# PaddlePaddle/PaddleNLP

Measured on NVIDIA H100. Metric: tokens/sec Llama-3.2-3B seq4096 bf16 pretrain step (global, all GPUs), higher is better.
Workload: dtype bf16

## Files before the change

paddlenlp_b200/csrc/gemm_wgmma.cu:

```cuda
#include "../../include/b200nlp.h"
#include <cstdlib>
#include <cstring>

#include "common.cuh"
#include "host_util.h"

namespace b200 {
namespace gemm {

constexpr int BN = 256;
constexpr int BK = 64;
constexpr int B_BYTES = BN * BK * 2;
constexpr int EPI_BOX = 64;
constexpr int EPI_BOX_BYTES = EPI_BOX * EPI_BOX * 2;
constexpr int EPI_BOX_F32 = 32;

template <int NWG>
struct Tile {
  static constexpr int BM = 64 * NWG;
  static constexpr int NUM_THREADS = 128 * (NWG + 1);
  static constexpr int A_BYTES = BM * BK * 2;
  static constexpr int STAGE_BYTES = A_BYTES + B_BYTES;
  static constexpr int STAGES = NWG == 2 ? 4 : 5;
  static constexpr int EPI_BYTES = NWG * 2 * EPI_BOX_BYTES;
  static constexpr int SMEM_BYTES = STAGES * STAGE_BYTES + EPI_BYTES + 256 + 1024;
};
static int tile_wgs(int64_t M) { return M <= 64 ? 1 : 2; }

struct Params {
  int M, N, K;
  int num_m_tiles, num_n_tiles;
  int epi_mode;
  int swiglu_inter;
  int gm;
  int split_k;
  int kb_per_split;
  const float* bias;
  bf16* c;
  int64_t ldc;
  const bf16* r;
  int64_t ldr;
  bf16* aux;
  int64_t ld_aux;
  float* ws;
};

__device__ __forceinline__ void fence_acc(float (&acc)[128]) {
#pragma unroll
  for (int i = 0; i < 128; ++i) asm volatile("" : "+f"(acc[i])::"memory");
}

__device__ __forceinline__ uint32_t epi_slot(uint32_t buf, int r, int jj, int lane) {
  return buf + r * 128 + ((jj ^ (r & 7)) << 4) + 4 * (lane & 3);
}
template <int KEEP>
__device__ __forceinline__ void epi_begin(int cw, bool leader) {
  if (leader) tma_store_wait_read<KEEP>();
  named_bar_sync(1 + cw, 128);
}
__device__ __forceinline__ void epi_end(int cw) {
  fence_proxy_async_smem();
  named_bar_sync(1 + cw, 128);
}
__device__ __forceinline__ uint32_t ld_pair(const bf16* base, int64_t ld, int row, int col, int M, int N) {
  if (row >= M || col >= N) return 0u;
  const bf16* src = base + static_cast<int64_t>(row) * ld + col;
  if (col + 1 < N) return *reinterpret_cast<const uint32_t*>(src);
  return static_cast<uint32_t>(__bfloat16_as_ushort(*src));
}
__device__ __forceinline__ void epi_prefetch(const CUtensorMap* tmC, const CUtensorMap* tmX, const Params& p, int n_blk, int row0) {
  for (int s = 0; s < BN / EPI_BOX; ++s) {
    const int col0 = n_blk * BN + EPI_BOX * s;
    if (col0 >= p.N) break;
    if (p.epi_mode == 1) {
      tma_prefetch_l2_2d(tmC, col0, row0);
    } else if (p.epi_mode == 2) {
      tma_prefetch_l2_2d(tmX, col0, row0);
    } else {
      tma_prefetch_l2_2d(tmX, col0, row0);
      tma_prefetch_l2_2d(tmX, p.swiglu_inter + col0, row0);
    }
  }
}

template <int NWG, bool A_MN, bool B_MN>
__global__ void __launch_bounds__(Tile<NWG>::NUM_THREADS, 1)
gemm_bf16_kernel(const __grid_constant__ CUtensorMap tmA, const __grid_constant__ CUtensorMap tmB,
                 const __grid_constant__ CUtensorMap tmC, const __grid_constant__ CUtensorMap tmX, const Params p) {
  using T = Tile<NWG>;
  constexpr int BM = T::BM, A_BYTES = T::A_BYTES, STAGE_BYTES = T::STAGE_BYTES, STAGES = T::STAGES;
  extern __shared__ uint8_t smem_raw[];
  uint8_t* smem = reinterpret_cast<uint8_t*>((reinterpret_cast<uintptr_t>(smem_raw) + 1023) & ~uintptr_t(1023));
  uint64_t* full_bar = reinterpret_cast<uint64_t*>(smem + STAGES * STAGE_BYTES + T::EPI_BYTES);
  uint64_t* empty_bar = full_bar + STAGES;

  const int num_items = p.num_m_tiles * p.num_n_tiles * p.split_k;
  const int num_kb_total = (p.K + BK - 1) / BK;
  if (threadIdx.x == 0) {
    tma_prefetch_desc(&tmA);
    tma_prefetch_desc(&tmB);
    for (int i = 0; i < STAGES; ++i) {
      mbar_init(&full_bar[i], 1);
      mbar_init(&empty_bar[i], NWG * 128);
    }
    fence_mbar_init();
  }
  __syncthreads();
  pdl_launch_dependents();
  pdl_wait();

  const int wg = threadIdx.x >> 7;
  if (wg == 0) {
    setmaxnreg_dec<40>();
    if (threadIdx.x == 0) {
      uint32_t it = 0;
      for (int t = blockIdx.x; t < num_items; t += gridDim.x) {
        int m_blk, n_blk;
        tile_coords(t / p.split_k, p.num_m_tiles, p.num_n_tiles, m_blk, n_blk, p.gm);
        const int kb0 = (t % p.split_k) * p.kb_per_split;
        const int kb1 = min(num_kb_total, kb0 + p.kb_per_split);
        for (int kb = kb0; kb < kb1; ++kb, ++it) {
          const int st = static_cast<int>(it % STAGES);
          mbar_wait_nocall(&empty_bar[st], ((it / STAGES) & 1u) ^ 1u);
          uint8_t* sA = smem + st * STAGE_BYTES;
          uint8_t* sB = sA + A_BYTES;
          mbar_arrive_expect_tx(&full_bar[st], STAGE_BYTES);
          if constexpr (A_MN) {
#pragma unroll
            for (int h = 0; h < NWG; ++h) tma_load_2d(&tmA, &full_bar[st], sA + h * (64 * BK * 2), m_blk * BM + 64 * h, kb * BK);
          } else {
            tma_load_2d(&tmA, &full_bar[st], sA, kb * BK, m_blk * BM);
          }
          if constexpr (B_MN) {
#pragma unroll
            for (int h = 0; h < 4; ++h) {
              const int c0 = p.epi_mode == 4 ? (h >> 1) * p.swiglu_inter + n_blk * 128 + (h & 1) * 64 : n_blk * BN + h * 64;
              tma_load_2d(&tmB, &full_bar[st], sB + h * (B_BYTES / 4), c0, kb * BK);
            }
          } else {
            tma_load_2d(&tmB, &full_bar[st], sB, kb * BK, n_blk * BN);
            tma_load_2d(&tmB, &full_bar[st], sB + B_BYTES / 2, kb * BK, n_blk * BN + 128);
          }
        }
      }
    }
    return;
  }

  setmaxnreg_inc<232>();
  const int cw = wg - 1;
  const int wi = (threadIdx.x >> 5) & 3, lane = threadIdx.x & 31;
  const uint32_t ring = smem_u32(smem);
  constexpr uint32_t A_KSTEP = A_MN ? 2048u : 32u, B_KSTEP = B_MN ? 2048u : 32u;
  const uint32_t a_off = static_cast<uint32_t>(cw) * (64 * BK * 2);
  const bool leader = (threadIdx.x & 127) == 0;
  const bool prefetch = leader && (p.epi_mode == 1 || p.epi_mode == 2 || p.epi_mode == 5);
  const uint32_t ebuf = smem_u32(smem + STAGES * STAGE_BYTES) + cw * 2 * EPI_BOX_BYTES;
  uint32_t nbox = 0;
  uint32_t it = 0;
  float acc[128];
  for (int t = blockIdx.x; t < num_items; t += gridDim.x) {
    int m_blk, n_blk;
    tile_coords(t / p.split_k, p.num_m_tiles, p.num_n_tiles, m_blk, n_blk, p.gm);
    const int kb0 = (t % p.split_k) * p.kb_per_split;
    const int nkb = min(num_kb_total, kb0 + p.kb_per_split) - kb0;
    const int prefetch_kb = nkb > 8 ? nkb - 8 : 0;
    fence_acc(acc);
#pragma unroll
    for (int i = 0; i < 128; ++i) acc[i] = 0.f;
    fence_acc(acc);
    for (int i = 0; i < nkb; ++i, ++it) {
      const int st = static_cast<int>(it % STAGES);
      mbar_wait_nocall(&full_bar[st], (it / STAGES) & 1u);
      const uint32_t sA = ring + st * STAGE_BYTES + a_off, sB = ring + st * STAGE_BYTES + A_BYTES;
      const uint64_t dA = wgmma_desc_sw128(sA, A_MN ? 64 * BK * 2 : 16, 1024);
      const uint64_t dB = wgmma_desc_sw128(sB, B_MN ? B_BYTES / 4 : 16, 1024);
      wgmma_fence();
#pragma unroll
      for (int kk = 0; kk < BK / 16; ++kk)
        wgmma_m64n256k16<A_MN ? 1 : 0, B_MN ? 1 : 0>(acc, dA + ((kk * A_KSTEP) >> 4), dB + ((kk * B_KSTEP) >> 4),
                                                     (i > 0 || kk > 0) ? 1u : 0u);
      wgmma_commit();
      if (prefetch && i == prefetch_kb) epi_prefetch(&tmC, &tmX, p, n_blk, m_blk * BM + cw * 64);
      wgmma_wait<1>();
      if (i > 0) mbar_arrive(&empty_bar[(it - 1) % STAGES]);
    }
    wgmma_wait<0>();
    fence_acc(acc);
    if (nkb > 0) mbar_arrive(&empty_bar[(it - 1) % STAGES]);

    const int row0 = m_blk * BM + cw * 64;
    const int r_lo = wi * 16 + (lane >> 2);
    const int cq = 2 * (lane & 3);
    if (p.epi_mode == 3) {
#pragma unroll
      for (int i = 0; i < 2; ++i) {
        const int row = row0 + r_lo + 8 * i;
        if (row >= p.M) continue;
#pragma unroll
        for (int j = 0; j < 32; ++j) {
          const int col = n_blk * BN + 8 * j + cq;
          if (col >= p.N) continue;
          float* w = p.ws + static_cast<int64_t>(row) * p.N + col;
          asm volatile("red.global.add.v2.f32 [%0], {%1, %2};" ::"l"(w), "f"(acc[4 * j + 2 * i]), "f"(acc[4 * j + 2 * i + 1])
                       : "memory");
        }
      }
      continue;
    }
    if (p.epi_mode == 4) {
#pragma unroll
      for (int h = 0; h < 2; ++h) {
        const int ch0 = n_blk * 128 + EPI_BOX * h;
        if (ch0 >= p.swiglu_inter) continue;
        if (p.aux != nullptr) {
          epi_begin<0>(cw, leader);
#pragma unroll
          for (int i = 0; i < 2; ++i)
#pragma unroll
            for (int jj = 0; jj < 8; ++jj) {
              const int j = 8 * h + jj;
              st_shared_u32(epi_slot(ebuf, r_lo + 8 * i, jj, lane), pack_bf16x2(acc[4 * j + 2 * i], acc[4 * j + 2 * i + 1]));
              st_shared_u32(epi_slot(ebuf + EPI_BOX_BYTES, r_lo + 8 * i, jj, lane),
                            pack_bf16x2(acc[4 * (j + 16) + 2 * i], acc[4 * (j + 16) + 2 * i + 1]));
            }
          epi_end(cw);
          if (leader) {
            tma_store_2d(&tmX, ebuf, ch0, row0);
            tma_store_2d(&tmX, ebuf + EPI_BOX_BYTES, p.swiglu_inter + ch0, row0);
            tma_store_commit();
          }
        }
        epi_begin<0>(cw, leader);
#pragma unroll
        for (int i = 0; i < 2; ++i)
#pragma unroll
          for (int jj = 0; jj < 8; ++jj) {
            const int j = 8 * h + jj;
            const uint32_t gp = pack_bf16x2(acc[4 * j + 2 * i], acc[4 * j + 2 * i + 1]);
            const uint32_t up = pack_bf16x2(acc[4 * (j + 16) + 2 * i], acc[4 * (j + 16) + 2 * i + 1]);
            st_shared_u32(epi_slot(ebuf, r_lo + 8 * i, jj, lane), swiglu_fwd_pair(gp, up));
          }
        epi_end(cw);
        if (leader) {
          tma_store_2d(&tmC, ebuf, ch0, row0);
          tma_store_commit();
        }
      }
      continue;
    }
    if (p.epi_mode == 5) {
#pragma unroll
      for (int s = 0; s < BN / EPI_BOX; ++s) {
        const int ch0 = n_blk * BN + EPI_BOX * s;
        if (ch0 >= p.N) continue;
        epi_begin<0>(cw, leader);
#pragma unroll
        for (int q = 0; q < 4; ++q) {
          const int i = q >> 1, jj0 = 4 * (q & 1);
          uint32_t g[4], u[4];
#pragma unroll
          for (int k = 0; k < 4; ++k) {
            const int row = row0 + r_lo + 8 * i, ch = ch0 + 8 * (jj0 + k) + cq;
            g[k] = ld_pair(p.aux, p.ld_aux, row, ch, p.M, p.N);
            u[k] = ld_pair(p.aux + p.swiglu_inter, p.ld_aux, row, ch, p.M, p.N);
          }
#pragma unroll
          for (int k = 0; k < 4; ++k) {
            const int jj = jj0 + k, j = 8 * s + jj;
            uint32_t dg2, du2;
            swiglu_bwd_pair(g[k], u[k], bf16_round(acc[4 * j + 2 * i]), bf16_round(acc[4 * j + 2 * i + 1]), dg2, du2);
            st_shared_u32(epi_slot(ebuf, r_lo + 8 * i, jj, lane), dg2);
            st_shared_u32(epi_slot(ebuf + EPI_BOX_BYTES, r_lo + 8 * i, jj, lane), du2);
          }
        }
        epi_end(cw);
        if (leader) {
          tma_store_2d(&tmC, ebuf, ch0, row0);
          tma_store_2d(&tmC, ebuf + EPI_BOX_BYTES, p.swiglu_inter + ch0, row0);
          tma_store_commit();
        }
      }
      continue;
    }
#pragma unroll
    for (int s = 0; s < BN / EPI_BOX; ++s) {
      const int col0 = n_blk * BN + EPI_BOX * s;
      if (col0 >= p.N) continue;
      if (p.epi_mode >= 6) {
        const uint32_t sw = (lane >> 2) << 4;
        const uint32_t row_off = r_lo * 128 + ((8 * (lane & 3)) ^ (sw & 16));
        epi_begin<0>(cw, leader);
#pragma unroll
        for (int h = 0; h < 2; ++h)
#pragma unroll
          for (int jj = 0; jj < 4; ++jj) {
            const int j = 8 * s + 4 * h + jj;
            const uint32_t slot = ebuf + h * EPI_BOX_BYTES + row_off + ((32 * jj) ^ (sw & 96));
            st_shared_f32x2(slot, acc[4 * j], acc[4 * j + 1]);
            st_shared_f32x2(slot + 8 * 128, acc[4 * j + 2], acc[4 * j + 3]);
          }
        epi_end(cw);
        if (leader) {
          if (p.epi_mode == 7) {
            tma_reduce_add_2d(&tmC, ebuf, col0, row0);
            tma_reduce_add_2d(&tmC, ebuf + EPI_BOX_BYTES, col0 + EPI_BOX_F32, row0);
          } else {
            tma_store_2d(&tmC, ebuf, col0, row0);
            tma_store_2d(&tmC, ebuf + EPI_BOX_BYTES, col0 + EPI_BOX_F32, row0);
          }
          tma_store_commit();
        }
        continue;
      }
      const uint32_t buf = ebuf + (nbox++ & 1u) * EPI_BOX_BYTES;
      epi_begin<1>(cw, leader);
#pragma unroll
      for (int i = 0; i < 2; ++i) {
        uint32_t o[8];
        if (p.epi_mode != 0) {
          const bf16* src = p.epi_mode == 1 ? p.c : p.r;
          const int64_t ld = p.epi_mode == 1 ? p.ldc : p.ldr;
#pragma unroll
          for (int jj = 0; jj < 8; ++jj) o[jj] = ld_pair(src, ld, row0 + r_lo + 8 * i, col0 + 8 * jj + cq, p.M, p.N);
        }
#pragma unroll
        for (int jj = 0; jj < 8; ++jj) {
          const int j = 8 * s + jj, col = col0 + 8 * jj + cq;
          float f0 = acc[4 * j + 2 * i], f1 = acc[4 * j + 2 * i + 1];
          if (p.bias != nullptr) {
            if (col < p.N) f0 += __ldg(p.bias + col);
            if (col + 1 < p.N) f1 += __ldg(p.bias + col + 1);
          }
          if (p.epi_mode != 0) {
            if (p.epi_mode == 2) { f0 = bf16_round(f0); f1 = bf16_round(f1); }
            const float2 of = unpack_bf16x2(o[jj]);
            f0 += of.x;
            f1 += of.y;
          }
          st_shared_u32(epi_slot(buf, r_lo + 8 * i, jj, lane), pack_bf16x2(f0, f1));
        }
      }
      epi_end(cw);
      if (leader) {
        tma_store_2d(&tmC, buf, col0, row0);
        tma_store_commit();
      }
    }
  }
  if (leader) tma_store_wait<0>();
}

template <int NWG, bool A_MN, bool B_MN>
static int launch(const CUtensorMap& tmA, const CUtensorMap& tmB, const CUtensorMap& tmC, const CUtensorMap& tmX, const Params& p,
                  int max_ctas, cudaStream_t stream) {
  using T = Tile<NWG>;
  constexpr int SMEM_BYTES = T::SMEM_BYTES;
  auto kern = gemm_bf16_kernel<NWG, A_MN, B_MN>;
  static bool attr_set = false;
  if (!attr_set) {
    cudaError_t e = cudaFuncSetAttribute(kern, cudaFuncAttributeMaxDynamicSharedMemorySize, SMEM_BYTES);
    if (e != cudaSuccess) {
      set_last_error("cudaFuncSetAttribute(gemm smem=%d): %s", SMEM_BYTES, cudaGetErrorString(e));
      return static_cast<int>(e);
    }
    attr_set = true;
  }
  const int num_items = p.num_m_tiles * p.num_n_tiles * p.split_k;
  int ctas = sm_count();
  if (max_ctas > 0 && max_ctas < ctas) ctas = max_ctas;
  if (ctas > num_items) ctas = num_items;
  Params pp = p;
  pp.gm = (16ll * 128 * p.K * 2 <= (18ll << 20)) ? 16 : 8;
  cudaError_t e = launch_pdl(kern, dim3(ctas), dim3(T::NUM_THREADS), SMEM_BYTES, stream, tmA, tmB, tmC, tmX, pp);
  if (e != cudaSuccess) {
    set_last_error("gemm launch: %s", cudaGetErrorString(e));
    return static_cast<int>(e);
  }
  return 0;
}

static int make_epi_map(CUtensorMap* tm, const void* base, int64_t rows, int64_t cols, int64_t ld) {
  const uint64_t dims[2] = {static_cast<uint64_t>(cols), static_cast<uint64_t>(rows)}, strides[1] = {static_cast<uint64_t>(ld) * 2};
  const uint32_t box[2] = {EPI_BOX, EPI_BOX};
  return encode_tmap_bf16(tm, base, 2, dims, strides, box);
}
static int make_epi_map_f32(CUtensorMap* tm, const void* base, int64_t rows, int64_t cols, int64_t ld) {
  const uint64_t dims[2] = {static_cast<uint64_t>(cols), static_cast<uint64_t>(rows)}, strides[1] = {static_cast<uint64_t>(ld) * 4};
  const uint32_t box[2] = {EPI_BOX_F32, EPI_BOX};
  return encode_tmap_f32(tm, base, 2, dims, strides, box);
}
static bool aligned16(const void* ptr) { return (reinterpret_cast<uintptr_t>(ptr) & 15) == 0; }

static int setup_smem_epilogue(const Params& p, CUtensorMap* tmC, CUtensorMap* tmX) {
  int rc;
  switch (p.epi_mode) {
    case 2:
      if ((rc = make_epi_map(tmX, p.r, p.M, p.N, p.ldr)) != 0) return rc;
      return make_epi_map(tmC, p.c, p.M, p.N, p.ldc);
    case 3:
      return 0;
    case 6:
    case 7:
      return make_epi_map_f32(tmC, p.ws, p.M, p.N, p.ldc);
    case 4:
      if (p.aux != nullptr && (rc = make_epi_map(tmX, p.aux, p.M, p.N, p.ld_aux)) != 0) return rc;
      return make_epi_map(tmC, p.c, p.M, p.swiglu_inter, p.ldc);
    case 5:
      if ((rc = make_epi_map(tmX, p.aux, p.M, 2ll * p.N, p.ld_aux)) != 0) return rc;
      return make_epi_map(tmC, p.c, p.M, 2ll * p.N, p.ldc);
    default:
      return make_epi_map(tmC, p.c, p.M, p.N, p.ldc);
  }
}

static int dispatch(bool a_mn, bool b_mn, const CUtensorMap& tmA, const CUtensorMap& tmB, Params p, int max_ctas,
                    cudaStream_t stream) {
  CUtensorMap tmC, tmX;
  memset(&tmC, 0, sizeof(tmC));
  memset(&tmX, 0, sizeof(tmX));
  int rc;
  if ((rc = setup_smem_epilogue(p, &tmC, &tmX)) != 0) return rc;
  if (tile_wgs(p.M) == 1) {
    if (a_mn && b_mn) return launch<1, true, true>(tmA, tmB, tmC, tmX, p, max_ctas, stream);
    if (a_mn) return launch<1, true, false>(tmA, tmB, tmC, tmX, p, max_ctas, stream);
    if (b_mn) return launch<1, false, true>(tmA, tmB, tmC, tmX, p, max_ctas, stream);
    return launch<1, false, false>(tmA, tmB, tmC, tmX, p, max_ctas, stream);
  }
  if (a_mn && b_mn) return launch<2, true, true>(tmA, tmB, tmC, tmX, p, max_ctas, stream);
  if (a_mn) return launch<2, true, false>(tmA, tmB, tmC, tmX, p, max_ctas, stream);
  if (b_mn) return launch<2, false, true>(tmA, tmB, tmC, tmX, p, max_ctas, stream);
  return launch<2, false, false>(tmA, tmB, tmC, tmX, p, max_ctas, stream);
}

static int make_a_map(CUtensorMap* tm, const void* A, int64_t M, int64_t K, int64_t lda, bool mn) {
  uint64_t dims[2], strides[1] = {static_cast<uint64_t>(lda) * 2};
  uint32_t box[2];
  if (mn) { dims[0] = M; dims[1] = K; box[0] = 64; box[1] = BK; }
  else    { dims[0] = K; dims[1] = M; box[0] = BK; box[1] = 64 * tile_wgs(M); }
  return encode_tmap_bf16(tm, A, 2, dims, strides, box);
}
static int make_b_map(CUtensorMap* tm, const void* B, int64_t N, int64_t K, int64_t ldb, bool mn) {
  uint64_t dims[2], strides[1] = {static_cast<uint64_t>(ldb) * 2};
  uint32_t box[2];
  if (mn) { dims[0] = N; dims[1] = K; box[0] = 64; box[1] = BK; }
  else    { dims[0] = K; dims[1] = N; box[0] = BK; box[1] = 128; }
  return encode_tmap_bf16(tm, B, 2, dims, strides, box);
}

static Params base_params(int64_t M, int64_t N, int64_t K) {
  Params p = {};
  p.M = static_cast<int>(M);
  p.N = static_cast<int>(N);
  p.K = static_cast<int>(K);
  const int64_t bm = 64 * tile_wgs(M);
  p.num_m_tiles = static_cast<int>((M + bm - 1) / bm);
  p.num_n_tiles = static_cast<int>((N + BN - 1) / BN);
  p.split_k = 1;
  p.kb_per_split = static_cast<int>((K + BK - 1) / BK);
  return p;
}

}
}

extern "C" int b200_gemm_bf16_ex(const void* A, const void* B, void* C, const float* bias, const void* residual,
                                 int64_t M, int64_t N, int64_t K, int64_t lda, int64_t ldb, int64_t ldc, int64_t ldr,
                                 int a_mn_major, int b_mn_major, int accumulate, int max_ctas, cudaStream_t stream) {
  using namespace b200;
  using namespace b200::gemm;
  B200_CHECK_ARG(A && B && C, "gemm: null pointer");
  B200_CHECK_ARG(M > 0 && N > 0 && K > 0, "gemm: non-positive dimension M=%lld N=%lld K=%lld", (long long)M,
                 (long long)N, (long long)K);
  B200_CHECK_ARG(lda % 8 == 0 && ldb % 8 == 0 && ldc % 8 == 0, "gemm: leading dimensions must be multiples of 8");
  B200_CHECK_ARG(!(residual && accumulate), "gemm: residual and accumulate are mutually exclusive");
  B200_CHECK_ARG(!residual || ldr % 8 == 0, "gemm: ldr must be a multiple of 8");
  B200_CHECK_ARG(M < (1ll << 31) && N < (1ll << 31) && K < (1ll << 31), "gemm: dimension too large");
  B200_CHECK_ARG(aligned16(C), "gemm: C must be 16-byte aligned");
  B200_CHECK_ARG(!residual || aligned16(residual), "gemm: residual must be 16-byte aligned");
  CUtensorMap tmA, tmB;
  int rc;
  if ((rc = make_a_map(&tmA, A, M, K, lda, a_mn_major)) != 0) return rc;
  if ((rc = make_b_map(&tmB, B, N, K, ldb, b_mn_major)) != 0) return rc;
  Params p = base_params(M, N, K);
  p.epi_mode = residual ? 2 : (accumulate ? 1 : 0);
  p.bias = bias;
  p.c = static_cast<bf16*>(C);
  p.ldc = ldc;
  p.r = static_cast<const bf16*>(residual);
  p.ldr = ldr;
  return dispatch(a_mn_major, b_mn_major, tmA, tmB, p, max_ctas, stream);
}

extern "C" int b200_gemm_bf16_f32(const void* A, const void* B, float* C, int64_t M, int64_t N, int64_t K, int64_t lda,
                                  int64_t ldb, int64_t ldc, int a_mn_major, int b_mn_major, int accumulate, cudaStream_t stream) {
  using namespace b200;
  using namespace b200::gemm;
  B200_CHECK_ARG(A && B && C, "gemm_f32: null pointer");
  B200_CHECK_ARG(M > 0 && N > 0 && K > 0, "gemm_f32: non-positive dimension M=%lld N=%lld K=%lld", (long long)M,
                 (long long)N, (long long)K);
  B200_CHECK_ARG(lda % 8 == 0 && ldb % 8 == 0, "gemm_f32: lda and ldb must be multiples of 8");
  B200_CHECK_ARG(ldc % 4 == 0 && ldc >= N, "gemm_f32: ldc must be a multiple of 4 and >= N (ldc=%lld N=%lld)", (long long)ldc,
                 (long long)N);
  B200_CHECK_ARG(M < (1ll << 31) && N < (1ll << 31) && K < (1ll << 31), "gemm_f32: dimension too large");
  B200_CHECK_ARG(aligned16(C), "gemm_f32: C must be 16-byte aligned");
  CUtensorMap tmA, tmB;
  int rc;
  if ((rc = make_a_map(&tmA, A, M, K, lda, a_mn_major)) != 0) return rc;
  if ((rc = make_b_map(&tmB, B, N, K, ldb, b_mn_major)) != 0) return rc;
  Params p = base_params(M, N, K);
  p.epi_mode = accumulate ? 7 : 6;
  p.ws = C;
  p.ldc = ldc;
  return dispatch(a_mn_major, b_mn_major, tmA, tmB, p, 0, stream);
}

extern "C" int b200_gemm_swiglu_bf16(const void* X, const void* W, void* GU, void* Mout, int64_t M, int64_t inter, int64_t K,
                                     int64_t ldx, int64_t ldw, int64_t ldgu, int64_t ldm, cudaStream_t stream) {
  using namespace b200;
  using namespace b200::gemm;
  B200_CHECK_ARG(X && W && Mout, "gemm_swiglu: null pointer");
  B200_CHECK_ARG(M > 0 && inter > 0 && K > 0 && inter % 64 == 0, "gemm_swiglu: intermediate size must be a multiple of 64 (got %lld)",
                 (long long)inter);
  B200_CHECK_ARG(ldx % 8 == 0 && ldw % 8 == 0 && ldgu % 8 == 0 && ldm % 8 == 0, "gemm_swiglu: leading dimensions must be multiples of 8");
  B200_CHECK_ARG(M < (1ll << 31) && inter < (1ll << 30) && K < (1ll << 31), "gemm_swiglu: dimension too large");
  B200_CHECK_ARG(aligned16(Mout), "gemm_swiglu: Mout must be 16-byte aligned");
  B200_CHECK_ARG(!GU || aligned16(GU), "gemm_swiglu: GU must be 16-byte aligned");
  CUtensorMap tmA, tmB;
  int rc;
  if ((rc = make_a_map(&tmA, X, M, K, ldx, false)) != 0) return rc;
  if ((rc = make_b_map(&tmB, W, 2 * inter, K, ldw, true)) != 0) return rc;
  Params p = base_params(M, 2 * inter, K);
  p.num_n_tiles = static_cast<int>((inter + 127) / 128);
  p.epi_mode = 4;
  p.swiglu_inter = static_cast<int>(inter);
  p.c = static_cast<bf16*>(Mout);
  p.ldc = ldm;
  p.aux = static_cast<bf16*>(GU);
  p.ld_aux = ldgu;
  return dispatch(false, true, tmA, tmB, p, 0, stream);
}

extern "C" int b200_gemm_swiglu_bwd_bf16(const void* dY, const void* Wdown, const void* GU, void* DGU, int64_t M, int64_t inter,
                                         int64_t K, int64_t lddy, int64_t ldw, int64_t ldgu, int64_t lddgu, cudaStream_t stream) {
  using namespace b200;
  using namespace b200::gemm;
  B200_CHECK_ARG(dY && Wdown && GU && DGU, "gemm_swiglu_bwd: null pointer");
  B200_CHECK_ARG(M > 0 && inter > 0 && K > 0 && inter % 64 == 0, "gemm_swiglu_bwd: intermediate size must be a multiple of 64 (got %lld)",
                 (long long)inter);
  B200_CHECK_ARG(lddy % 8 == 0 && ldw % 8 == 0 && ldgu % 8 == 0 && lddgu % 8 == 0, "gemm_swiglu_bwd: leading dimensions must be multiples of 8");
  B200_CHECK_ARG(M < (1ll << 31) && inter < (1ll << 30) && K < (1ll << 31), "gemm_swiglu_bwd: dimension too large");
  B200_CHECK_ARG(aligned16(GU), "gemm_swiglu_bwd: GU must be 16-byte aligned");
  B200_CHECK_ARG(aligned16(DGU), "gemm_swiglu_bwd: DGU must be 16-byte aligned");
  CUtensorMap tmA, tmB;
  int rc;
  if ((rc = make_a_map(&tmA, dY, M, K, lddy, false)) != 0) return rc;
  if ((rc = make_b_map(&tmB, Wdown, inter, K, ldw, false)) != 0) return rc;
  Params p = base_params(M, inter, K);
  p.epi_mode = 5;
  p.swiglu_inter = static_cast<int>(inter);
  p.c = static_cast<bf16*>(DGU);
  p.ldc = lddgu;
  p.aux = const_cast<bf16*>(static_cast<const bf16*>(GU));
  p.ld_aux = ldgu;
  return dispatch(false, false, tmA, tmB, p, 0, stream);
}

namespace b200 {
namespace gemm {
__global__ void splitk_finish_kernel(float* __restrict__ ws, const float* __restrict__ bias, bf16* __restrict__ out,
                                     int64_t M, int64_t N, int64_t ldc) {
  const int64_t nch = N >> 3;
  const int64_t total = M * nch;
  for (int64_t i = blockIdx.x * static_cast<int64_t>(blockDim.x) + threadIdx.x; i < total;
       i += static_cast<int64_t>(gridDim.x) * blockDim.x) {
    const int64_t r = i / nch, c = i % nch;
    float4* src = reinterpret_cast<float4*>(ws + r * N) + 2 * c;
    float4 a = src[0], b = src[1];
    src[0] = make_float4(0.f, 0.f, 0.f, 0.f);
    src[1] = make_float4(0.f, 0.f, 0.f, 0.f);
    if (bias != nullptr) {
      const float4* bp = reinterpret_cast<const float4*>(bias) + 2 * c;
      const float4 b0 = __ldg(bp), b1 = __ldg(bp + 1);
      a.x += b0.x; a.y += b0.y; a.z += b0.z; a.w += b0.w;
      b.x += b1.x; b.y += b1.y; b.z += b1.z; b.w += b1.w;
    }
    uint4 o;
    o.x = pack_bf16x2(a.x, a.y); o.y = pack_bf16x2(a.z, a.w);
    o.z = pack_bf16x2(b.x, b.y); o.w = pack_bf16x2(b.z, b.w);
    *(reinterpret_cast<uint4*>(out + r * ldc) + c) = o;
  }
}
}

int splitk_finish(float* ws, const float* bias, void* out, int64_t M, int64_t N, int64_t ldc, cudaStream_t stream) {
  const int64_t total = M * (N / 8);
  int64_t blocks = (total + 255) / 256;
  if (blocks > sm_count() * 8) blocks = sm_count() * 8;
  gemm::splitk_finish_kernel<<<static_cast<unsigned>(blocks), 256, 0, stream>>>(ws, bias, static_cast<bf16*>(out), M, N, ldc);
  return check_launch("gemm_splitk(finish)");
}

}

extern "C" int64_t b200_gemm_splitk_workspace_bytes(int64_t M, int64_t N) { return M * N * 4; }

extern "C" int b200_gemm_bf16_splitk(const void* A, const void* B, void* C, const float* bias, void* workspace, int64_t M,
                                     int64_t N, int64_t K, int64_t lda, int64_t ldb, int64_t ldc, int a_mn_major,
                                     int b_mn_major, int split_k, cudaStream_t stream) {
  using namespace b200;
  using namespace b200::gemm;
  B200_CHECK_ARG(A && B && workspace, "gemm_splitk: null pointer");
  B200_CHECK_ARG(M > 0 && N > 0 && K > 0 && N % 8 == 0, "gemm_splitk: bad dimensions (N must be a multiple of 8)");
  B200_CHECK_ARG(lda % 8 == 0 && ldb % 8 == 0 && ldc % 8 == 0, "gemm_splitk: leading dimensions must be multiples of 8");
  B200_CHECK_ARG(!C || aligned16(C), "gemm_splitk: C must be 16-byte aligned");
  CUtensorMap tmA, tmB;
  int rc;
  if ((rc = make_a_map(&tmA, A, M, K, lda, a_mn_major)) != 0) return rc;
  if ((rc = make_b_map(&tmB, B, N, K, ldb, b_mn_major)) != 0) return rc;
  Params p = base_params(M, N, K);
  const int num_kb = p.kb_per_split;
  const int tiles = p.num_m_tiles * p.num_n_tiles;
  if (split_k <= 0) {
    const int sms = sm_count();
    split_k = (sms + tiles - 1) / tiles;
    if (split_k > num_kb / 4) split_k = num_kb / 4;
    if (split_k < 1) split_k = 1;
  }
  p.kb_per_split = (num_kb + split_k - 1) / split_k;
  p.split_k = (num_kb + p.kb_per_split - 1) / p.kb_per_split;
  p.epi_mode = 3;
  p.ws = static_cast<float*>(workspace);
  if ((rc = dispatch(a_mn_major, b_mn_major, tmA, tmB, p, 0, stream)) != 0) return rc;
  if (C == nullptr) return 0;
  return splitk_finish(static_cast<float*>(workspace), bias, C, M, N, ldc, stream);
}

extern "C" int b200_gemm_bf16(const void* A, const void* B, void* C, const float* bias, int64_t M, int64_t N, int64_t K,
                              int64_t lda, int64_t ldb, int64_t ldc, int a_mn_major, int b_mn_major, int accumulate,
                              cudaStream_t stream) {
  return b200_gemm_bf16_ex(A, B, C, bias, nullptr, M, N, K, lda, ldb, ldc, 0, a_mn_major, b_mn_major, accumulate,
                           0, stream);
}
```

Before: 23700.

## Stage GEMM epilogue residual/C inputs through TMA loads into shared memory

For epilogue modes that add a residual or existing C tile, the kernel now issues TMA loads of the input boxes into the epilogue shared buffers. The first loads start during the last K-blocks of the mainloop, and later boxes are double-buffered behind each TMA store, tracked by new per-warpgroup mbarriers. The values are then read back from shared memory in place, replacing per-thread global ld_pair loads. This aims to hide epilogue global-load latency and coalesce the traffic. In exchange it adds barrier and phase bookkeeping, store-read waits, and extra smem barrier space that is not clearly budgeted. It also relies on the TMA box layout matching the epi_slot swizzle.

```diff
diff --git a/paddlenlp_b200/csrc/gemm_wgmma.cu b/paddlenlp_b200/csrc/gemm_wgmma.cu
--- a/paddlenlp_b200/csrc/gemm_wgmma.cu
+++ b/paddlenlp_b200/csrc/gemm_wgmma.cu
@@ -83,6 +83,17 @@
   }
 }
 
+__device__ __forceinline__ void epi_load_box(const CUtensorMap* tm, uint64_t* bar, uint8_t* dst, const Params& p, int col0, int row0) {
+  if (col0 >= p.N) return;
+  mbar_arrive_expect_tx(bar, EPI_BOX_BYTES);
+  tma_load_2d(tm, bar, dst, col0, row0);
+}
+__device__ __forceinline__ uint32_t ld_shared_u32(uint32_t saddr) {
+  uint32_t v;
+  asm volatile("ld.shared.u32 %0, [%1];" : "=r"(v) : "r"(saddr));
+  return v;
+}
+
 template <int NWG, bool A_MN, bool B_MN>
 __global__ void __launch_bounds__(Tile<NWG>::NUM_THREADS, 1)
 gemm_bf16_kernel(const __grid_constant__ CUtensorMap tmA, const __grid_constant__ CUtensorMap tmB,
@@ -93,6 +104,7 @@
   uint8_t* smem = reinterpret_cast<uint8_t*>((reinterpret_cast<uintptr_t>(smem_raw) + 1023) & ~uintptr_t(1023));
   uint64_t* full_bar = reinterpret_cast<uint64_t*>(smem + STAGES * STAGE_BYTES + T::EPI_BYTES);
   uint64_t* empty_bar = full_bar + STAGES;
+  uint64_t* epi_bar = empty_bar + STAGES;
 
   const int num_items = p.num_m_tiles * p.num_n_tiles * p.split_k;
   const int num_kb_total = (p.K + BK - 1) / BK;
@@ -103,6 +115,7 @@
       mbar_init(&full_bar[i], 1);
       mbar_init(&empty_bar[i], NWG * 128);
     }
+    for (int i = 0; i < 2 * NWG; ++i) mbar_init(&epi_bar[i], 1);
     fence_mbar_init();
   }
   __syncthreads();
@@ -155,8 +168,12 @@
   const uint32_t a_off = static_cast<uint32_t>(cw) * (64 * BK * 2);
   const bool leader = (threadIdx.x & 127) == 0;
   const bool prefetch = leader && (p.epi_mode == 1 || p.epi_mode == 2 || p.epi_mode == 5);
-  const uint32_t ebuf = smem_u32(smem + STAGES * STAGE_BYTES) + cw * 2 * EPI_BOX_BYTES;
+  uint8_t* const ebuf_p = smem + STAGES * STAGE_BYTES + cw * 2 * EPI_BOX_BYTES;
+  const uint32_t ebuf = smem_u32(ebuf_p);
   uint32_t nbox = 0;
+  const bool tma_in = p.epi_mode == 1 || p.epi_mode == 2;
+  const CUtensorMap* tm_in = p.epi_mode == 1 ? &tmC : &tmX;
+  uint32_t eph = 0;
   uint32_t it = 0;
   float acc[128];
   for (int t = blockIdx.x; t < num_items; t += gridDim.x) {
@@ -181,7 +198,15 @@
         wgmma_m64n256k16<A_MN ? 1 : 0, B_MN ? 1 : 0>(acc, dA + ((kk * A_KSTEP) >> 4), dB + ((kk * B_KSTEP) >> 4),
                                                      (i > 0 || kk > 0) ? 1u : 0u);
       wgmma_commit();
-      if (prefetch && i == prefetch_kb) epi_prefetch(&tmC, &tmX, p, n_blk, m_blk * BM + cw * 64);
+      if (prefetch && i == prefetch_kb) {
+        epi_prefetch(&tmC, &tmX, p, n_blk, m_blk * BM + cw * 64);
+        if (tma_in) {
+          tma_store_wait_read<0>();
+#pragma unroll
+          for (int b = 0; b < 2; ++b) epi_load_box(tm_in, &epi_bar[2 * cw + b], ebuf_p + b * EPI_BOX_BYTES, p, n_blk * BN + EPI_BOX * b,
+                                                   m_blk * BM + cw * 64);
+        }
+      }
       wgmma_wait<1>();
       if (i > 0) mbar_arrive(&empty_bar[(it - 1) % STAGES]);
     }
@@ -313,17 +338,17 @@
         }
         continue;
       }
-      const uint32_t buf = ebuf + (nbox++ & 1u) * EPI_BOX_BYTES;
-      epi_begin<1>(cw, leader);
+      uint32_t buf;
+      if (tma_in) {
+        buf = ebuf + (s & 1) * EPI_BOX_BYTES;
+        mbar_wait_nocall(&epi_bar[2 * cw + (s & 1)], (eph >> (s & 1)) & 1u);
+        eph ^= 1u << (s & 1);
+      } else {
+        buf = ebuf + (nbox++ & 1u) * EPI_BOX_BYTES;
+        epi_begin<1>(cw, leader);
+      }
 #pragma unroll
       for (int i = 0; i < 2; ++i) {
-        uint32_t o[8];
-        if (p.epi_mode != 0) {
-          const bf16* src = p.epi_mode == 1 ? p.c : p.r;
-          const int64_t ld = p.epi_mode == 1 ? p.ldc : p.ldr;
-#pragma unroll
-          for (int jj = 0; jj < 8; ++jj) o[jj] = ld_pair(src, ld, row0 + r_lo + 8 * i, col0 + 8 * jj + cq, p.M, p.N);
-        }
 #pragma unroll
         for (int jj = 0; jj < 8; ++jj) {
           const int j = 8 * s + jj, col = col0 + 8 * jj + cq;
@@ -332,9 +357,9 @@
             if (col < p.N) f0 += __ldg(p.bias + col);
             if (col + 1 < p.N) f1 += __ldg(p.bias + col + 1);
           }
-          if (p.epi_mode != 0) {
+          if (tma_in) {
             if (p.epi_mode == 2) { f0 = bf16_round(f0); f1 = bf16_round(f1); }
-            const float2 of = unpack_bf16x2(o[jj]);
+            const float2 of = unpack_bf16x2(ld_shared_u32(epi_slot(buf, r_lo + 8 * i, jj, lane)));
             f0 += of.x;
             f1 += of.y;
           }
@@ -345,6 +370,10 @@
       if (leader) {
         tma_store_2d(&tmC, buf, col0, row0);
         tma_store_commit();
+        if (tma_in && s + 2 < BN / EPI_BOX) {
+          tma_store_wait_read<0>();
+          epi_load_box(tm_in, &epi_bar[2 * cw + (s & 1)], ebuf_p + (s & 1) * EPI_BOX_BYTES, p, col0 + 2 * EPI_BOX, row0);
+        }
       }
     }
   }
```

Result: faster. 24070 (median of 6 runs) (+1.5%).
